# AIS-Bonn/stillleben

Hardware: AMD Instinct MI355X
Metric: scenes/sec (settle + 640x480 6-ch GT render), 20-obj YCB-like (higher is better)
Workload: dtype f32; 1 GPU; C2: 20 of 21 procedural YCB-like objects (8k verts/16k tris, 1024^2 texture each) per scene; per step and GPU 32768 scenes are staged (random stack), settled (100 frames x 4 substeps), framed (camera, light, shadow matrix) and rendered at 640x480 (rgb, coord+depth, class, instance, normals; shadows on, SSAO on) -- all four stages inside the timed region; render_chunk=512, objects=20, settle_streams=1, render_streams=2, pair_contact_budget=0, parallelism=1 GPU

## Files before the change

### include/slhip.h

```cpp
#ifndef SLHIP_H
#define SLHIP_H

#include <stdint.h>

#ifdef __cplusplus
extern "C" {
#endif

#define SLHIP_ABI_VERSION 5
#define SLHIP_NUM_LIGHTS 3


typedef struct {
    float* d_env;
    float* d_irradiance;
    float* d_prefilter;
    float* d_brdf_lut;
    uint32_t env_size, env_levels;
    uint32_t irr_size;
    uint32_t pre_size, pre_levels;
    uint32_t lut_size;
} slhip_light_map;

typedef struct {
// ... 105 lines not shown
} slhip_render_out;

typedef struct {
    uint64_t* d_vis;
    float*    d_hdr;
    float*    d_ao;
    float*    d_shadow;
    uint32_t* d_queue;
    float*    d_lum;
    float*    d_clip;
    uint32_t* d_shadow_tiles;
    uint32_t  queue_capacity;
    uint32_t  shadow_res;
    uint32_t  n_clip_verts;
    uint32_t  shadow_lights;
    float*    d_vattr;
} slhip_render_scratch;

int slhip_render(const slhip_mesh_pool* pool,
                 const slhip_scene* d_scenes, const slhip_draw* d_draws,
                 const slhip_chunk* d_chunks, uint32_t n_scenes, uint32_t n_draws, uint32_t n_chunks,
                 uint32_t width, uint32_t height, uint32_t flags,
                 const float* d_depth_peel,
                 const slhip_render_out* out, const slhip_render_scratch* scratch,
                 void* stream);

int slhip_timing_enable(int on);
int slhip_render_timings(float* ms_out);
int slhip_render_ssao_skipped(const slhip_render_scratch* scratch, uint32_t n_scenes, uint32_t width, uint32_t height,
                              uint64_t counts[2], void* stream);
int slhip_render_ssao_level_tables(float rho[5], uint32_t counts[6], uint8_t taps[384]);
int slhip_render_ssao_levels(const slhip_render_scratch* scratch, uint32_t n_scenes, uint32_t width, uint32_t height,
                             uint64_t counts[8], void* stream);

int slhip_render_scratch_bytes(uint32_t n_scenes, uint32_t width, uint32_t height,
                               uint32_t shadow_res, uint32_t queue_capacity,
                               uint64_t bytes_out[7]);

typedef struct {
    uint32_t px_visib, px_all;
    int32_t  bbox_visib[4];
    int32_t  bbox_obj[4];
} slhip_object_stats;

#define SLHIP_OBJECT_STATS_CAPACITY 1

int slhip_render_object_stats_bytes(uint32_t n_scenes, uint32_t n_slots, uint32_t width, uint32_t height,
                                    uint64_t* worst_case_words);

int slhip_render_object_stats(const slhip_mesh_pool* pool,
                              const slhip_scene* d_scenes, const slhip_draw* d_draws,
                              const slhip_chunk* d_chunks, uint32_t n_scenes, uint32_t n_draws, uint32_t n_chunks,
                              uint32_t width, uint32_t height, const slhip_render_scratch* scratch,
                              uint32_t n_slots, uint64_t* d_words, uint64_t capacity_words,
                              slhip_object_stats* d_out, uint64_t* words_needed, void* stream);

typedef struct {
    int32_t  tile_box[4];
    uint64_t word_offset[2];
    uint64_t rle_offset[2];
    uint32_t rle_count[2];
} slhip_object_mask;

#define SLHIP_OBJECT_MASKS_CAPACITY 2

int slhip_render_object_masks_bytes(uint32_t n_scenes, uint32_t n_slots, uint32_t width, uint32_t height,
// ... 675 lines not shown
```

### stillleben_amd/_abi.py

```python
import ctypes as C
import os

import numpy as np

NUM_LIGHTS = 3
CHUNK_TRIS = 256

DRAW_HAS_BASE_TEX = 1
DRAW_VERTEX_COLORS = 2
DRAW_CASTS_SHADOW = 4
DRAW_ALPHA_TEST = 8
DRAW_NO_VERTEX_ID = 16
DRAW_HAS_NORMAL_TEX = 32
DRAW_HAS_MR_TEX = 64
DRAW_HAS_OCCLUSION_TEX = 128
DRAW_HAS_EMISSIVE_TEX = 256
DRAW_HAS_STICKER = 512
SAMPLER_DEFAULT = 0x10 | 0x20 | (2 << 6)

OUT_RGB = 0x01
OUT_COORD = 0x02
OUT_CLASS = 0x04
OUT_INSTANCE = 0x08
OUT_NORMALS = 0x10
# ... 407 lines not shown
    L.slhip_render_timings.argtypes = [C.POINTER(C.c_float * 8)]
    L.slhip_diff_sobel_valid.argtypes = [C.c_void_p, C.c_void_p, C.c_int, C.c_int, C.c_int, C.c_void_p, C.c_void_p]
    L.slhip_diff_dilate.argtypes = [C.c_void_p, C.c_void_p, C.c_void_p, C.c_int, C.c_int, C.c_int, C.c_void_p, C.c_void_p, C.c_void_p]
    L.slhip_diff_image_gradients.argtypes = [C.c_void_p, C.c_void_p, C.c_int, C.c_int, C.c_void_p, C.c_void_p, C.c_void_p]
    L.slhip_diff_pose_backward.argtypes = [C.c_void_p] * 7 + [C.c_int, C.c_int, C.c_int] + [C.c_void_p] * 4
    L.slhip_diff_pose_backward_batch.argtypes = [C.c_void_p] * 4 + [C.c_uint64] + [C.c_void_p] * 3 + [C.c_int] * 4 + [C.c_void_p] * 4
    L.slhip_diff_vertex_backward.argtypes = [C.c_void_p] * 8 + [C.c_int, C.c_int, C.c_int] + [C.c_void_p] * 4
    L.slhip_settle.argtypes = [C.c_void_p, C.c_uint32, C.c_void_p, C.c_void_p, C.c_void_p, C.c_void_p,
                               C.c_void_p, C.c_uint64, C.c_void_p]
    L.slhip_settle_status.argtypes = [C.c_void_p, C.c_uint32, C.c_void_p, C.POINTER(C.c_uint32), C.c_void_p]
    L.slhip_host_shadow_matrices.argtypes = [C.c_void_p, C.c_void_p, C.c_void_p]
    L.slhip_host_normal_matrix.argtypes = [C.c_void_p, C.c_void_p]
    L.slhip_host_convex_hull.argtypes = [C.c_void_p, C.c_uint32, C.c_void_p, C.c_uint32, C.POINTER(C.c_uint32)]
    L.slhip_host_fill_holes.argtypes = [C.c_void_p, C.c_uint32, C.c_uint32, C.c_uint32]
    L.slhip_records_count.argtypes = [C.c_void_p, C.c_uint32, C.c_void_p, C.c_void_p, C.POINTER(C.c_uint32), C.POINTER(C.c_uint32)]
    L.slhip_records_build_render.argtypes = [C.c_void_p, C.c_uint32, C.c_void_p, C.c_void_p, C.c_uint32, C.c_void_p, C.c_void_p,
                                             C.c_uint32, C.c_void_p, C.c_uint32]
    L.slhip_render_object_stats.argtypes = [
        C.POINTER(MeshPool), C.c_void_p, C.c_void_p, C.c_void_p, C.c_uint32, C.c_uint32, C.c_uint32, C.c_uint32, C.c_uint32,
        C.POINTER(RenderScratch), C.c_uint32, C.c_void_p, C.c_uint64, C.c_void_p, C.POINTER(C.c_uint64), C.c_void_p,
    ]
    L.slhip_render_object_stats_bytes.argtypes = [C.c_uint32, C.c_uint32, C.c_uint32, C.c_uint32, C.POINTER(C.c_uint64)]
    L.slhip_render_object_masks.argtypes = [
        C.POINTER(MeshPool), C.c_void_p, C.c_void_p, C.c_void_p, C.c_uint32, C.c_uint32, C.c_uint32, C.c_uint32, C.c_uint32,
        C.POINTER(RenderScratch), C.c_uint32, C.c_void_p, C.c_uint64, C.c_void_p, C.POINTER(C.c_uint64),
        C.c_void_p, C.c_void_p, C.c_uint64, C.POINTER(C.c_uint64), C.c_void_p,
    ]
    L.slhip_render_object_masks_bytes.argtypes = [C.c_uint32, C.c_uint32, C.c_uint32, C.c_uint32, C.POINTER(C.c_uint64),
                                                  C.POINTER(C.c_uint64)]
    L.slhip_object_masks_expand.argtypes = [C.c_void_p, C.c_void_p, C.c_uint32, C.c_uint32, C.c_uint32, C.c_uint32, C.c_uint32,
                                            C.c_void_p, C.c_uint64, C.c_void_p, C.c_void_p]
    L.slhip_render_ssao_skipped.argtypes = [C.c_void_p, C.c_uint32, C.c_uint32, C.c_uint32, C.POINTER(C.c_uint64 * 2), C.c_void_p]
    L.slhip_render_ssao_levels.argtypes = [C.c_void_p, C.c_uint32, C.c_uint32, C.c_uint32, C.POINTER(C.c_uint64 * 8), C.c_void_p]
    L.slhip_render_ssao_level_tables.argtypes = [C.POINTER(C.c_float * 5), C.POINTER(C.c_uint32 * 6), C.POINTER(C.c_uint8 * 384)]
    L.slhip_settle_caps.argtypes = [C.c_void_p, C.c_uint32, C.c_void_p, C.POINTER(C.c_uint64 * 10), C.c_void_p]
    L.slhip_settle_timing_enable.argtypes = [C.c_int]
    L.slhip_settle_timings.argtypes = [C.POINTER(C.c_float * 5), C.POINTER(C.c_uint32 * 5)]
    if hasattr(L, "slhip_settle_timing_every"):
        L.slhip_settle_timing_every.argtypes = [C.c_uint32]
        L.slhip_settle_timings_by_step.argtypes = [C.c_void_p, C.c_void_p, C.c_uint32, C.POINTER(C.c_uint32)]
    L.slhip_settle_scratch_bytes.argtypes = [C.c_uint32, C.c_void_p, C.POINTER(C.c_uint64)]
    L.slhip_overlap_any.argtypes = [C.c_void_p, C.c_uint32, C.c_void_p, C.c_void_p, C.c_void_p, C.c_void_p, C.c_void_p]
    L.slhip_light_map_floats.argtypes = [C.c_uint32] * 6 + [C.POINTER(C.c_uint64 * 4)]
    L.slhip_light_map_build.argtypes = [C.c_void_p, C.c_int, C.c_int, C.c_void_p, C.c_void_p]
    L.slhip_camera_model.argtypes = [C.c_void_p, C.c_void_p, C.c_void_p, C.c_uint32, C.c_int, C.c_int, C.c_void_p, C.c_void_p]
    if hasattr(L, "slhip_depth_sensor"):
        L.slhip_depth_sensor_check_params.argtypes = [C.c_void_p, C.c_uint32, C.c_int]
        L.slhip_depth_sensor_timing_enable.argtypes = [C.c_int]
        L.slhip_depth_sensor_timings.argtypes = [C.POINTER(C.c_float * 2)]
        L.slhip_depth_sensor_scratch_bytes.argtypes = [C.c_uint32, C.c_int, C.c_int, C.POINTER(C.c_uint64)]
        L.slhip_depth_sensor.argtypes = [C.c_void_p, C.c_uint32, C.c_void_p, C.c_uint32, C.c_uint32, C.c_int, C.c_int, C.c_void_p,
                                         C.c_void_p, C.c_void_p, C.c_void_p, C.c_void_p, C.c_void_p]
    if hasattr(L, "slhip_object_crops_select"):
        L.slhip_object_crops_check_params.argtypes = [C.c_void_p, C.c_int, C.c_int]
        L.slhip_object_crops_scratch_bytes.argtypes = [C.c_uint32, C.POINTER(C.c_uint64)]
        L.slhip_object_crops_select.argtypes = [C.c_void_p, C.c_void_p, C.c_uint32, C.c_uint32, C.c_int, C.c_int, C.c_void_p,
                                                C.c_uint64, C.c_void_p, C.POINTER(C.c_uint64), C.c_void_p]
        L.slhip_object_crops_gather.argtypes = [C.c_void_p, C.c_void_p, C.c_uint64, C.POINTER(RenderOut), C.c_uint32, C.c_int,
                                                C.c_int, C.c_void_p, C.c_void_p, C.c_uint32, C.POINTER(ObjectCropsOut), C.c_void_p]
        L.slhip_object_crops_timing_enable.argtypes = [C.c_int]
        L.slhip_object_crops_timings.argtypes = [C.POINTER(C.c_float * 2)]
    if hasattr(L, "slhip_object_points_select"):
        L.slhip_object_points_check_params.argtypes = [C.c_void_p, C.c_int, C.c_int]
        L.slhip_object_points_scratch_bytes.argtypes = [C.c_uint32, C.POINTER(C.c_uint64)]
        L.slhip_object_points_select.argtypes = [C.c_void_p, C.c_void_p, C.c_void_p, C.c_uint32, C.c_uint32, C.c_void_p,
                                                 C.c_uint64, C.c_void_p, C.POINTER(C.c_uint64), C.c_void_p]
# ... 90 lines not shown
```

### stillleben_amd/_engine.py

```python
import ctypes as C

import numpy as np
import torch

from . import _abi
from ._batch import HostPool, build_batch

SHADOW_RES = 2048
QUEUE_ITEMS_PER_SCENE = int(__import__('os').environ.get('SLHIP_QUEUE_ITEMS', 1 << 14))


def _ptr(t):
    return C.c_void_p(t.data_ptr()) if t is not None else C.c_void_p(0)


class RenderBuffers:

    def __init__(self, device, B, H, W, mask):
        self.B, self.H, self.W, self.mask = B, H, W, mask

        def mk(bit, shape, dtype):
            return torch.empty(shape, dtype=dtype, device=device) if mask & bit else None

        self.rgb = mk(_abi.OUT_RGB, (B, H, W, 4), torch.uint8)
# ... 80 lines not shown
                "shadow_ready": False,
            }
            if len(self._scratch) > 6:
                self._scratch.clear()
            self._scratch[key] = s
        a = _abi.RenderScratch()
        a.d_vis, a.d_hdr, a.d_ao, a.d_shadow, a.d_queue, a.d_lum = (
            _ptr(s["vis"]), _ptr(s["hdr"]), _ptr(s["ao"]), _ptr(s["shadow"]), _ptr(s["queue"]), _ptr(s["lum"]))
        a.d_shadow_tiles = _ptr(s["tiles"])
        a.queue_capacity = s["qcap"]
        a.shadow_res = SHADOW_RES
        a.shadow_lights = shadow_lights
        return a, s

    def ssao_skipped(self, buffers, W, H):
        keep = buffers._keepalive[0]
        a = _abi.RenderScratch()
        a.d_ao = _ptr(keep["ao"])
        out = (C.c_uint64 * 2)()
        stream = torch.cuda.current_stream(self.device).cuda_stream
        with torch.cuda.device(self.device):
            _abi.check(self.L.slhip_render_ssao_skipped(C.byref(a), buffers.B, W, H, C.byref(out), C.c_void_p(stream)), "slhip_render_ssao_skipped")
        return int(out[0]), int(out[1])

    def ssao_levels(self, buffers, W, H):
        keep = buffers._keepalive[0]
        a = _abi.RenderScratch()
        a.d_ao = _ptr(keep["ao"])
        out = (C.c_uint64 * 8)()
        stream = torch.cuda.current_stream(self.device).cuda_stream
        with torch.cuda.device(self.device):
            _abi.check(self.L.slhip_render_ssao_levels(C.byref(a), buffers.B, W, H, C.byref(out), C.c_void_p(stream)), "slhip_render_ssao_levels")
        return [int(v) for v in out[:6]], int(out[6]), int(out[7])

    def upload_records(self, arr):
        raw = np.frombuffer(arr.tobytes(), dtype=np.uint8) if arr.size else np.zeros(16, np.uint8)
        return torch.from_numpy(raw.copy()).to(self.device)

    def render(self, scenes, mask=_abi.OUT_ALL, ssao=True, shadows=True, depth_peel=None, predicate=None,
               buffers=None, keep_hdr=False, object_stats=False, object_masks=False):
        W, H = scenes[0]._viewport
        for s in scenes:
            if s._viewport != (W, H):
                raise ValueError("all scenes of a batch must share one viewport")
        if (object_stats or object_masks) and depth_peel is not None:
            raise ValueError("object_stats / object_masks cannot be combined with depth_peel: a peeled layer has no single whole silhouette")
        n_slots = None
        if object_stats or object_masks:
            n_slots = 1 + max((int(o.instance_index) for s in scenes for o in s._objects), default=0)
        want_rgb = bool(mask & _abi.OUT_RGB)
        srec, drec, crec = build_batch(scenes, self.pool, predicate, with_shadows=shadows and want_rgb)
        return self.render_records(srec, drec, crec, W, H, mask, ssao, shadows, depth_peel, buffers, keep_hdr,
                                   object_stats=object_stats, n_slots=n_slots, object_masks=object_masks)

    def render_records(self, srec, drec, crec, W, H, mask=_abi.OUT_ALL, ssao=True, shadows=True, depth_peel=None,
                       buffers=None, keep_hdr=False, object_stats=False, n_slots=None, stats_capacity=None,
                       object_masks=False, masks_capacity=None):
        if (object_stats or object_masks) and n_slots is None:
            n_slots = 1 + (int((drec["instance_index"] & 0xFFFF).max()) if len(drec) else 0)
        d_s, d_d, d_c = self.upload_records(srec), self.upload_records(drec), self.upload_records(crec)
        n_clip = int(drec["n_verts"].sum()) if len(drec) else 0
        on = (np.abs(srec["light_color"][:, :, :3]).sum(axis=2) > 0) & (np.abs(srec["light_dir"][:, :, :3]).sum(axis=2) > 0)
        lights = max(1, int(np.max(np.nonzero(on.any(axis=0))[0]) + 1)) if on.any() else 1
        buffers = self.render_device(d_s, d_d, d_c, len(srec), len(drec), len(crec), n_clip, W, H, mask, ssao, shadows,
                                     depth_peel, buffers, keep_hdr, shadow_lights=lights, object_stats=object_stats,
                                     n_slots=n_slots, stats_capacity=stats_capacity, object_masks=object_masks,
# ... 116 lines not shown
```

### stillleben_amd/csrc/slhip_render.hip

```cpp
#include <algorithm>
#include <cmath>
#include <cstring>
#include <vector>
#include <type_traits>
#include "slhip_common.h"
#include "slhip_cubemap.h"
#include "slhip_raster_walk.h"
#include "slhip_tile_queue.h"

#ifndef SLHIP_RENDER_WAVES
#define SLHIP_RENDER_WAVES 0
#endif
#ifndef SLHIP_SHADE_WAVES
#define SLHIP_SHADE_WAVES 0
#endif
#ifndef SLHIP_SSAO_WAVES
#define SLHIP_SSAO_WAVES 0
#endif
#if SLHIP_RENDER_WAVES > 0
#define SLHIP_LIGHT_KERNEL __attribute__((amdgpu_waves_per_eu(1, SLHIP_RENDER_WAVES)))
#else
#define SLHIP_LIGHT_KERNEL
#endif
#if SLHIP_RENDER_WAVES > 0
#define SLHIP_SHADOW_RASTER_KERNEL SLHIP_LIGHT_KERNEL
#else
#define SLHIP_SHADOW_RASTER_KERNEL __attribute__((amdgpu_waves_per_eu(6)))
#endif
#if SLHIP_SSAO_WAVES > 0
#define SLHIP_SSAO_KERNEL __attribute__((amdgpu_waves_per_eu(1, SLHIP_SSAO_WAVES)))
#else
#define SLHIP_SSAO_KERNEL
#endif
#if SLHIP_SHADE_WAVES > 0
#define SLHIP_SHADE_KERNEL __attribute__((amdgpu_waves_per_eu(1, SLHIP_SHADE_WAVES)))
#else
#define SLHIP_SHADE_KERNEL
#endif
namespace {

// ... 1980 lines not shown
        for (; k < n_taps; ++k) tap(k);
    }
    };
    if (w_is_z) taps(std::true_type{});
    else taps(std::false_type{});
    return 1.0f - occlusion / 64.0f;
}

__global__ __launch_bounds__(256) SLHIP_SSAO_KERNEL void k_ssao(const slhip_scene* __restrict__ scenes, unsigned n_scenes, int W, int H,
                                              const float* __restrict__ cam, const float* __restrict__ nrm,
                                              const float* __restrict__ zplane, float* __restrict__ ao,
                                              const float* __restrict__ kern)
{
    const size_t P = (size_t)W * H;
    const unsigned blocks_per_scene = (unsigned)((P + 255) / 256);
    unsigned scene, blk;
    if (!scene_block(blocks_per_scene, n_scenes, scene, blk)) return;
    const unsigned pix = blk * 256 + (threadIdx.x >> 6) + 4u * (threadIdx.x & 63u);
    if (pix >= P) return;
    const float* proj = scenes[scene].proj;
    const float* camS = zplane + (size_t)scene * ((size_t)(W + 2) * (H + 2));
    const size_t gp = (size_t)scene * P + pix;
    const int i = (int)(pix % (unsigned)W), j = (int)(pix / (unsigned)W);
    const float4 n4 = reinterpret_cast<const float4*>(nrm)[gp];
    if (n4.x == 0.0f && n4.y == 0.0f && n4.z == 0.0f) { ao[gp] = 1.0f; return; }
    ao[gp] = ssao_pixel<true>(proj, camS, W, H, i, j, n4, reinterpret_cast<const float4*>(cam)[gp], kern);
}

constexpr int kSsaoTile = 8;
constexpr int kSsaoLevels = 6;
constexpr float kSsaoRho[kSsaoLevels - 1] = {0.81f, 0.6f, 0.45f, 0.3f, 0.2f};
__constant__ float c_ssao_level_kernel[kSsaoLevels * 192];
struct SsaoLevelCounts { int n[kSsaoLevels]; };

__global__ __launch_bounds__(256) void k_ssao_mask(const slhip_scene* __restrict__ scenes, int W, int H,
                                                  const float2* __restrict__ tiles, unsigned char* __restrict__ skip, int dbg,
                                                  unsigned* __restrict__ drain_stats)
{
    extern __shared__ int s_sat[];
    const int TW = W / kSsaoTile, TH = H / kSsaoTile, SW = TW + 1;
    const unsigned scene = blockIdx.x;
    const float2* T = tiles + (size_t)scene * (TW * TH);
    unsigned char* S = skip + (size_t)scene * (TW * TH);
    const float* proj = scenes[scene].proj;
    if (scene == 0 && threadIdx.x < 2) drain_stats[threadIdx.x] = 0u;
    const bool persp = proj[1] == 0.0f && proj[3] == 0.0f && proj[4] == 0.0f && proj[7] == 0.0f &&
                       proj[12] == 0.0f && proj[13] == 0.0f && proj[14] == 1.0f && proj[15] == 0.0f && proj[0] > 0.0f && proj[5] > 0.0f;
    for (int k = threadIdx.x; k < (TH + 1) * SW; k += 256) {
        const int r = k / SW, c = k % SW;
        s_sat[k] = (r > 0 && c > 0) ? (int)(__float_as_uint(T[(r - 1) * TW + (c - 1)].y) & 1u) : 0;
    }
    __syncthreads();
    for (int r = threadIdx.x + 1; r <= TH; r += 256) { int acc = 0; for (int c = 1; c <= TW; ++c) { acc += s_sat[r * SW + c]; s_sat[r * SW + c] = acc; } }
    __syncthreads();
    for (int c = threadIdx.x + 1; c <= TW; c += 256) { int acc = 0; for (int r = 1; r <= TH; ++r) { acc += s_sat[r * SW + c]; s_sat[r * SW + c] = acc; } }
    __syncthreads();
    const float fx = proj[0] * 0.5f * (float)W, fy = proj[5] * 0.5f * (float)H;
    const float tx = (1.0f + fabsf(proj[2])) / proj[0], ty = (1.0f + fabsf(proj[6])) / proj[5];
    const float tmax = fmaxf(tx, ty);
    const float reach = fmaxf(fx, fy) * 0.1f * sqrtf(1.0f + tmax * tmax) * 1.001f;
    for (int k = threadIdx.x; k < TW * TH; k += 256) {
        const float2 t = T[k];
        const unsigned fl = __float_as_uint(t.y);
        int lvl = kSsaoLevels - 1, pass = 0;
        if (!(fl & 2u)) { lvl = 0; pass = 1; }
        else if (persp && !(fl & 1u) && t.x > 0.2f) {
            for (int j = kSsaoLevels - 2; j >= -1; --j) {
                const int R = (int)ceilf((j >= 0 ? kSsaoRho[j] : 1.0f) * reach / (t.x - 0.1f)) + 2;
                const int x0 = (k % TW) * kSsaoTile - R, x1 = (k % TW) * kSsaoTile + kSsaoTile - 1 + R;
                const int y0 = (k / TW) * kSsaoTile - R, y1 = (k / TW) * kSsaoTile + kSsaoTile - 1 + R;
                if (!(x0 >= 0 && y0 >= 0 && x1 < W && y1 < H)) break;
                const int ca = x0 / kSsaoTile, cb = x1 / kSsaoTile + 1, ra = y0 / kSsaoTile, rb = y1 / kSsaoTile + 1;
                const int others = s_sat[rb * SW + cb] - s_sat[ra * SW + cb] - s_sat[rb * SW + ca] + s_sat[ra * SW + ca];
                if (others != 0) break;
                if (j >= 0) lvl = j;
                else pass = 1;
            }
        }
        if (dbg == 1) { lvl = 0; pass = 1; }
        if (dbg == 2) lvl = kSsaoLevels - 1;
        S[k] = (unsigned char)(lvl << 1 | pass);
    }
}

__global__ __launch_bounds__(256) SLHIP_SSAO_KERNEL void k_ssao_tiled(const slhip_scene* __restrict__ scenes, unsigned n_scenes, int W, int H,
                                                    const float* __restrict__ cam, const float* __restrict__ nrm,
                                                    const float* __restrict__ zplane, float* __restrict__ ao,
                                                    const float* __restrict__ level_kern, SsaoLevelCounts level_n,
                                                    const unsigned char* __restrict__ skip, unsigned band_rows,
                                                    unsigned* __restrict__ drain_stats)
{
    __shared__ unsigned s_q[4][kSsaoLevels - 1][128];
    const unsigned bands = ((unsigned)H + band_rows - 1u) / band_rows;
    unsigned scene, rest;
    if (!scene_block(bands * 4u, n_scenes, scene, rest)) return;
    const unsigned band = rest >> 2, yc = rest & 3u, xc = threadIdx.x >> 6, lane = threadIdx.x & 63u;
    const size_t P = (size_t)W * H;
    const float* proj = scenes[scene].proj;
    const float* camS = zplane + (size_t)scene * ((size_t)(W + 2) * (H + 2));
    const int TW = W / kSsaoTile;
    const unsigned char* S = skip + (size_t)scene * ((size_t)TW * (H / kSsaoTile));
    const float4* N4 = reinterpret_cast<const float4*>(nrm) + (size_t)scene * P;
    const float4* C4 = reinterpret_cast<const float4*>(cam) + (size_t)scene * P;
    float* A = ao + (size_t)scene * P;
    unsigned* q = &s_q[xc][0][0];
    const unsigned y_first = band * band_rows, rows = min(band_rows, (unsigned)H - y_first);
    const unsigned per_row = (unsigned)W >> 2, total = (rows >> 2) * per_row;
    unsigned cnt[kSsaoLevels] = {};
    auto pixel_of = [&](unsigned ci) -> unsigned { return (y_first + yc + 4u * (ci / per_row)) * (unsigned)W + xc + 4u * (ci % per_row); };
    auto fetch = [&](unsigned ci, unsigned& pix, unsigned& lvl, float4& n4) {
        pix = 0; lvl = 0; n4 = make_float4(0.0f, 0.0f, 0.0f, 0.0f);
        if (ci < total) {
            pix = pixel_of(ci);
            const unsigned y = pix / (unsigned)W, x = pix % (unsigned)W;
            const unsigned b = S[(y >> 3) * (unsigned)TW + (x >> 3)];
            lvl = min(b >> 1, (unsigned)(kSsaoLevels - 1));
            if (lvl) n4 = N4[pix];
        }
    };
    unsigned pix_n, lvl_n; float4 n4_n;
    fetch(lane, pix_n, lvl_n, n4_n);
    unsigned c0 = 0;
    for (;;) {
        unsigned pix = 0, list = 0;
        bool valid = false;
#pragma unroll
        for (int l = 1; l < kSsaoLevels; ++l)
            if (cnt[l] >= 64u) list = (unsigned)l;
        if (list) {
#pragma unroll
            for (int l = 1; l < kSsaoLevels; ++l)
                if (list == (unsigned)l) { cnt[l] -= 64u; pix = q[(l - 1) * 128 + cnt[l] + lane]; }
            valid = true;
        } else if (c0 < total) {
            const unsigned px = pix_n, lvl = lvl_n;
            const float4 n4 = n4_n;
            const bool in = c0 + lane < total;
            c0 += 64u;
            fetch(c0 + lane, pix_n, lvl_n, n4_n);
            const bool need = in && lvl != 0u && !(n4.x == 0.0f && n4.y == 0.0f && n4.z == 0.0f);
            if (in && !need) A[px] = 1.0f;
#pragma unroll
            for (int l = 1; l < kSsaoLevels; ++l) {
                const bool mine = need && lvl == (unsigned)l;
                const unsigned long long m = __ballot(mine);
                if (mine) q[(l - 1) * 128 + cnt[l] + (unsigned)__popcll(m & ((1ull << lane) - 1ull))] = px;
                cnt[l] += (unsigned)__popcll(m);
            }
            __builtin_amdgcn_wave_barrier();
            continue;
        } else {
            unsigned room = 64u, p = lane, lowest = 0;
#pragma unroll
            for (int l = kSsaoLevels - 1; l >= 1; --l) {
                const unsigned take = min(cnt[l], room);
                if (take) {
                    if (!list) list = (unsigned)l;
                    lowest = (unsigned)l;
                    cnt[l] -= take;
                    room -= take;
                    if (!valid) {
                        if (p < take) { pix = q[(l - 1) * 128 + cnt[l] + p]; valid = true; }
                        else p -= take;
                    }
                }
            }
            if (!list) break;
            if (drain_stats && lane == 0u) {
                atomicAdd(&drain_stats[0], 1u);
                if (lowest != list) atomicAdd(&drain_stats[1], 1u);
            }
        }
        __builtin_amdgcn_wave_barrier();
        int n_taps = 0;
#pragma unroll
        for (int l = 1; l < kSsaoLevels; ++l)
            if (list == (unsigned)l) n_taps = level_n.n[l];
        if (valid) {
            const int i = (int)(pix % (unsigned)W), j = (int)(pix / (unsigned)W);
            A[pix] = ssao_pixel(proj, camS, W, H, i, j, N4[pix], C4[pix], level_kern + 192u * list, n_taps);
        }
        __builtin_amdgcn_wave_barrier();
    }
}

__global__ __launch_bounds__(256) SLHIP_LIGHT_KERNEL void k_ssao_apply(const slhip_scene* __restrict__ scenes, unsigned n_scenes, int W, int H,
                                                    const float* __restrict__ hdr_in, const float* __restrict__ ao,
                                                    const float* __restrict__ zplane, float* __restrict__ hdr_out,
                                                    const float* __restrict__ lum_scene, uint8_t* __restrict__ rgb,
                                                    const unsigned char* __restrict__ skip)
{
    const size_t P = (size_t)W * H;
    const unsigned blocks_per_scene = (unsigned)((P + 255) / 256);
    unsigned scene, blk;
    if (!scene_block(blocks_per_scene, n_scenes, scene, blk)) return;
    const unsigned pix = blk * 256 + threadIdx.x;
    if (pix >= P) return;
    const float* camS = zplane + (size_t)scene * ((size_t)(W + 2) * (H + 2));
    const float* aoS = ao + (size_t)scene * P;
    const size_t gp = (size_t)scene * P + pix;
    const int i = (int)(pix % (unsigned)W), j = (int)(pix / (unsigned)W);
    if (skip) {
        const int TW = W / kSsaoTile;
        const unsigned char* S = skip + (size_t)scene * ((size_t)TW * (H / kSsaoTile));
        const int xa = max(i - 2, 0) >> 3, xb = min(i + 1, W - 1) >> 3, ya = max(j - 2, 0) >> 3, yb = min(j + 1, H - 1) >> 3;
        const bool ones = (S[ya * TW + xa] & S[ya * TW + xb] & S[yb * TW + xa] & S[yb * TW + xb] & 1) != 0;
        if (__all(ones)) {
            const float4 h = reinterpret_cast<const float4*>(hdr_in)[gp];
            const float c4[4] = {h.x, h.y, h.z, h.w};
            if (hdr_out) reinterpret_cast<float4*>(hdr_out)[gp] = h;
            if (rgb) {
                const float manual = scenes[scene].manual_exposure;
                const float lum = (manual >= 0.0f) ? 0.0f : lum_scene[(size_t)scene * blocks_per_scene * 4];
                reinterpret_cast<uchar4*>(rgb)[gp] = tone_map_px(c4, manual, lum);
            }
// ... 176 lines not shown
                if (j < kSsaoLevels - 1 && !(1.001 * std::sqrt(x * x + y * y + z * z) > (double)kSsaoRho[j])) continue;
                for (int c = 0; c < 3; ++c) t.kern[j * 192 + 3 * n + c] = k_ssao_kernel_host[3 * k + c];
                t.taps[j * 64 + n] = (uint8_t)k;
                ++n;
            }
            t.count.n[j] = n;
        }
        return t;
    }();
    return tables;
}
}

extern "C" int slhip_render_ssao_level_tables(float rho[5], uint32_t counts[6], uint8_t taps[384])
{
    if (!rho || !counts || !taps) {
        slhip::set_error("slhip_render_ssao_level_tables: null argument");
        return -1;
    }
    const SsaoLevelTables& t = ssao_level_tables();
    for (int j = 0; j < kSsaoLevels - 1; ++j) rho[j] = kSsaoRho[j];
    for (int j = 0; j < kSsaoLevels; ++j) counts[j] = (uint32_t)t.count.n[j];
    memcpy(taps, t.taps, sizeof(t.taps));
    return 0;
}

static inline uint64_t ssao_tiles_per_scene(uint32_t w, uint32_t h) { return (uint64_t)((w + 7) / 8) * ((h + 7) / 8); }
static inline uint64_t ssao_tiles_offset(uint64_t B, uint32_t w, uint32_t h)
{
    const uint64_t b = B * (uint64_t)w * h * 4 + B * (uint64_t)(w + 2) * (h + 2) * 4;
    return (b + 7u) & ~(uint64_t)7u;
}

constexpr uint64_t kSsaoScratchSpare = 16;
static_assert(7 + 2 * sizeof(unsigned) <= kSsaoScratchSpare, "the two counters of k_ssao_tiled, 8-byte aligned, live in the spare bytes");
static inline uint64_t ssao_stats_offset(uint64_t B, uint32_t w, uint32_t h)
{
    return (ssao_tiles_offset(B, w, h) + B * ssao_tiles_per_scene(w, h) * 9 + 7u) & ~(uint64_t)7u;
}

extern "C" int slhip_render_scratch_bytes(uint32_t n_scenes, uint32_t width, uint32_t height,
                                          uint32_t shadow_res, uint32_t queue_capacity, uint64_t bytes_out[7])
{
    const uint64_t P = (uint64_t)width * height, B = n_scenes;
    const uint64_t blocks = (P + 255) / 256;
    bytes_out[0] = B * P * 8;
    bytes_out[1] = 2 * B * P * 16;
    bytes_out[2] = ssao_tiles_offset(B, width, height) + B * ssao_tiles_per_scene(width, height) * 9 + kSsaoScratchSpare;
    bytes_out[3] = B * SLHIP_NUM_LIGHTS * (uint64_t)shadow_res * shadow_res * 4;
    bytes_out[4] = 16 + (uint64_t)queue_capacity * 16;
    bytes_out[5] = B * blocks * 16;
    bytes_out[6] = B * SLHIP_NUM_LIGHTS * (uint64_t)shadow_tile_words((int)shadow_res) * 4;
    return 0;
}

extern "C" int slhip_render_ssao_skipped(const slhip_render_scratch* scratch, uint32_t n_scenes, uint32_t width, uint32_t height,
                                         uint64_t counts[2], void* stream_)
{
    hipStream_t stream = (hipStream_t)stream_;
    if (!scratch || !scratch->d_ao || !counts) {
        slhip::set_error("slhip_render_ssao_skipped: null argument");
        return -1;
    }
    counts[0] = counts[1] = 0;
    if (width % 32 != 0 || height % 16 != 0 || n_scenes == 0) return 0;
    const uint64_t nt = (uint64_t)n_scenes * ssao_tiles_per_scene(width, height);
    std::vector<unsigned char> h(nt);
    const char* base = reinterpret_cast<const char*>(scratch->d_ao) + ssao_tiles_offset(n_scenes, width, height) + nt * 8;
    SLHIP_CHECK(hipMemcpyAsync(h.data(), base, nt, hipMemcpyDeviceToHost, stream));
    SLHIP_CHECK(hipStreamSynchronize(stream));
    counts[0] = nt;
    for (unsigned char b : h) counts[1] += b & 1;
    return 0;
}

extern "C" int slhip_render_ssao_levels(const slhip_render_scratch* scratch, uint32_t n_scenes, uint32_t width, uint32_t height,
                                        uint64_t counts[8], void* stream_)
{
    hipStream_t stream = (hipStream_t)stream_;
    if (!scratch || !scratch->d_ao || !counts) {
        slhip::set_error("slhip_render_ssao_levels: null argument");
        return -1;
    }
    for (int i = 0; i < 8; ++i) counts[i] = 0;
    if (width % 32 != 0 || height % 16 != 0 || n_scenes == 0) return 0;
    const uint64_t nt = (uint64_t)n_scenes * ssao_tiles_per_scene(width, height);
    std::vector<unsigned char> h(nt);
    unsigned stats[2] = {0, 0};
    const char* ao = reinterpret_cast<const char*>(scratch->d_ao);
    SLHIP_CHECK(hipMemcpyAsync(h.data(), ao + ssao_tiles_offset(n_scenes, width, height) + nt * 8, nt, hipMemcpyDeviceToHost, stream));
    SLHIP_CHECK(hipMemcpyAsync(stats, ao + ssao_stats_offset(n_scenes, width, height), sizeof(stats), hipMemcpyDeviceToHost, stream));
    SLHIP_CHECK(hipStreamSynchronize(stream));
    for (unsigned char b : h) counts[std::min<int>(b >> 1, kSsaoLevels - 1)] += 1;
    counts[6] = stats[0];
    counts[7] = stats[1];
    return 0;
}

constexpr int kSsaoBandRows = 16;
static unsigned ssao_band_rows_knob()
{
    const char* e = getenv("SLHIP_SSAO_BAND_ROWS");
    const int v = e ? atoi(e) : kSsaoBandRows;
    return (unsigned)std::min(std::max(16, v / 16 * 16), 1 << 16);
}

extern "C" int slhip_render(const slhip_mesh_pool* pool, const slhip_scene* d_scenes, const slhip_draw* d_draws,
                            const slhip_chunk* d_chunks, uint32_t n_scenes, uint32_t n_draws, uint32_t n_chunks,
                            uint32_t width,
                            uint32_t height, uint32_t flags, const float* d_depth_peel,
                            const slhip_render_out* out, const slhip_render_scratch* scratch, void* stream_)
{
    hipStream_t stream = (hipStream_t)stream_;
    if (!pool || !d_scenes || !d_draws || !out || !scratch) {
        slhip::set_error("slhip_render: null argument");
        return -1;
    }
    if (n_scenes == 0 || width == 0 || height == 0) return 0;
    if (!scratch->d_vis || !scratch->d_queue) {
        slhip::set_error("slhip_render: d_vis and d_queue scratch are required");
        return -1;
    }
    const bool want_rgb = out->d_rgb != nullptr;
    const bool ssao = (flags & SLHIP_RENDER_SSAO) && want_rgb;
    const bool shadows = (flags & SLHIP_RENDER_SHADOWS) && want_rgb && scratch->d_shadow != nullptr;
    if (shadows && (!scratch->d_shadow_tiles || (scratch->shadow_res & 3u))) {
        slhip::set_error("slhip_render: shadows need the d_shadow_tiles scratch and a shadow_res that is a multiple of 4");
        return -1;
// ... 123 lines not shown
    float2* ssao_tiles = ssao_tiled ? reinterpret_cast<float2*>(reinterpret_cast<char*>(scratch->d_ao) + ssao_tiles_offset(n_scenes, W, H)) : nullptr;
    unsigned char* ssao_skip = ssao_tiled ? reinterpret_cast<unsigned char*>(ssao_tiles + (size_t)n_scenes * ssao_tiles_per_scene(W, H)) : nullptr;
    const int shade_reference = getenv("SLHIP_SHADE_REFERENCE") ? atoi(getenv("SLHIP_SHADE_REFERENCE")) : 0;
    auto launch_shade = [&](auto kernel) {
        kernel<<<pix_blocks, 256, 0, stream>>>(*pool, d_scenes, d_draws, prm,
                                               reinterpret_cast<const unsigned long long*>(scratch->d_vis), *out, hdr0,
                                               shadows ? scratch->d_shadow : nullptr, scratch->d_lum, clipbuf,
                                               ssao ? scratch->d_ao + (size_t)n_scenes * P : nullptr, vattr, ssao_tiles,
                                               shadows && !getenv("SLHIP_NO_PCF_TILES") ? scratch->d_shadow_tiles : nullptr);
    };
    if (shade_reference) launch_shade(k_shade<true>);
    else launch_shade(k_shade<false>);
    SLHIP_LAUNCH_CHECK();
    if (shadows && n_chunks > 0) {
        k_shadow_restore<<<n_tile_words, 256, 0, stream>>>(reinterpret_cast<unsigned*>(scratch->d_shadow), scratch->d_shadow_tiles,
                                                          S, n_tile_words, NL);
        SLHIP_LAUNCH_CHECK();
    }

    if (want_rgb) {
        k_lum_reduce<<<n_scenes, 256, 0, stream>>>(d_scenes, (unsigned)((P + 255) / 256), P, scratch->d_lum);
        if (ssao) {
            mark(5, stream);
            const float* zpl = scratch->d_ao + (size_t)n_scenes * P;
            const float* d_kernel_table = nullptr;
            SLHIP_CHECK(hipGetSymbolAddress((void**)&d_kernel_table, HIP_SYMBOL(c_ssao_kernel)));
            if (ssao_tiled) {
                const unsigned band_rows = ssao_band_rows_knob();
                const int ssao_dbg = getenv("SLHIP_SSAO_DEBUG") ? atoi(getenv("SLHIP_SSAO_DEBUG")) : 0;
                const unsigned bands = ((unsigned)H + band_rows - 1u) / band_rows;
                unsigned* drain_stats = reinterpret_cast<unsigned*>(reinterpret_cast<char*>(scratch->d_ao) + ssao_stats_offset(n_scenes, W, H));
                const float* d_level_table = nullptr;
                SLHIP_CHECK(hipGetSymbolAddress((void**)&d_level_table, HIP_SYMBOL(c_ssao_level_kernel)));
                k_ssao_mask<<<n_scenes, 256, (size_t)(W / 8 + 1) * (H / 8 + 1) * 4, stream>>>(d_scenes, W, H, ssao_tiles, ssao_skip, ssao_dbg, drain_stats);
                k_ssao_tiled<<<8u * ((n_scenes + 7u) / 8u) * bands * 4u, 256, 0, stream>>>(d_scenes, n_scenes, W, H, out->d_cam_coord, out->d_normals,
                                                                                   zpl, scratch->d_ao, d_level_table, ssao_level_tables().count, ssao_skip,
                                                                                   band_rows, ssao_dbg == 3 ? drain_stats : nullptr);
            } else
                k_ssao<<<pix_blocks, 256, 0, stream>>>(d_scenes, n_scenes, W, H, out->d_cam_coord, out->d_normals, zpl, scratch->d_ao,
                                                       d_kernel_table);
            mark(6, stream);
            k_ssao_apply<<<pix_blocks, 256, 0, stream>>>(d_scenes, n_scenes, W, H, hdr0, scratch->d_ao, zpl,
                                                         (flags & SLHIP_RENDER_KEEP_HDR) ? hdr1 : nullptr, scratch->d_lum, out->d_rgb, ssao_skip);
            mark(7, stream);
        } else {
            mark(7, stream);
            k_tonemap<<<pix_blocks, 256, 0, stream>>>(d_scenes, n_scenes, W, H, hdr0, scratch->d_lum, out->d_rgb);
        }
        SLHIP_LAUNCH_CHECK();
    }
    mark(kNumPhases, stream);
    return 0;
}

#include "slhip_render_stats.inc"
#include "slhip_render_masks.inc"
```

Before: 11110 scenes/s.

## Pool leftover SSAO queue tails across waves in a block before draining

In the tiled SSAO kernel, each wave no longer drains its own partial per-level pixel queues. Instead, all four waves publish their leftover counts to shared memory, synchronise, and then cooperatively process the pooled leftovers as full 64-lane batches ordered by level. This is meant to reduce partially filled wave iterations and mixed-level drains at the tail of each band, at the cost of a block-wide barrier and extra indexing work. The change also skips the enqueue ballots when no lane needs SSAO, and adds debug counters plus a host query for run-slot statistics.

```diff
diff --git a/include/slhip.h b/include/slhip.h
--- a/include/slhip.h
+++ b/include/slhip.h
@@ -161,6 +161,8 @@
 int slhip_render_ssao_level_tables(float rho[5], uint32_t counts[6], uint8_t taps[384]);
 int slhip_render_ssao_levels(const slhip_render_scratch* scratch, uint32_t n_scenes, uint32_t width, uint32_t height,
                              uint64_t counts[8], void* stream);
+int slhip_render_ssao_run_slots(const slhip_render_scratch* scratch, uint32_t n_scenes, uint32_t width, uint32_t height,
+                                uint64_t slots[4], void* stream);
 
 int slhip_render_scratch_bytes(uint32_t n_scenes, uint32_t width, uint32_t height,
                                uint32_t shadow_res, uint32_t queue_capacity,
diff --git a/stillleben_amd/_abi.py b/stillleben_amd/_abi.py
--- a/stillleben_amd/_abi.py
+++ b/stillleben_amd/_abi.py
@@ -463,6 +463,7 @@
                                             C.c_void_p, C.c_uint64, C.c_void_p, C.c_void_p]
     L.slhip_render_ssao_skipped.argtypes = [C.c_void_p, C.c_uint32, C.c_uint32, C.c_uint32, C.POINTER(C.c_uint64 * 2), C.c_void_p]
     L.slhip_render_ssao_levels.argtypes = [C.c_void_p, C.c_uint32, C.c_uint32, C.c_uint32, C.POINTER(C.c_uint64 * 8), C.c_void_p]
+    L.slhip_render_ssao_run_slots.argtypes = [C.c_void_p, C.c_uint32, C.c_uint32, C.c_uint32, C.POINTER(C.c_uint64 * 4), C.c_void_p]
     L.slhip_render_ssao_level_tables.argtypes = [C.POINTER(C.c_float * 5), C.POINTER(C.c_uint32 * 6), C.POINTER(C.c_uint8 * 384)]
     L.slhip_settle_caps.argtypes = [C.c_void_p, C.c_uint32, C.c_void_p, C.POINTER(C.c_uint64 * 10), C.c_void_p]
     L.slhip_settle_timing_enable.argtypes = [C.c_int]
diff --git a/stillleben_amd/_engine.py b/stillleben_amd/_engine.py
--- a/stillleben_amd/_engine.py
+++ b/stillleben_amd/_engine.py
@@ -136,6 +136,16 @@
         with torch.cuda.device(self.device):
             _abi.check(self.L.slhip_render_ssao_levels(C.byref(a), buffers.B, W, H, C.byref(out), C.c_void_p(stream)), "slhip_render_ssao_levels")
         return [int(v) for v in out[:6]], int(out[6]), int(out[7])
+
+    def ssao_run_slots(self, buffers, W, H):
+        keep = buffers._keepalive[0]
+        a = _abi.RenderScratch()
+        a.d_ao = _ptr(keep["ao"])
+        out = (C.c_uint64 * 4)()
+        stream = torch.cuda.current_stream(self.device).cuda_stream
+        with torch.cuda.device(self.device):
+            _abi.check(self.L.slhip_render_ssao_run_slots(C.byref(a), buffers.B, W, H, C.byref(out), C.c_void_p(stream)), "slhip_render_ssao_run_slots")
+        return tuple(int(v) for v in out)
 
     def upload_records(self, arr):
         raw = np.frombuffer(arr.tobytes(), dtype=np.uint8) if arr.size else np.zeros(16, np.uint8)
diff --git a/stillleben_amd/csrc/slhip_render.hip b/stillleben_amd/csrc/slhip_render.hip
--- a/stillleben_amd/csrc/slhip_render.hip
+++ b/stillleben_amd/csrc/slhip_render.hip
@@ -6,6 +6,7 @@
 #include "slhip_common.h"
 #include "slhip_cubemap.h"
 #include "slhip_raster_walk.h"
+#include "slhip_ssao_pool.h"
 #include "slhip_tile_queue.h"
 
 #ifndef SLHIP_RENDER_WAVES
@@ -2052,6 +2053,7 @@
 constexpr float kSsaoRho[kSsaoLevels - 1] = {0.81f, 0.6f, 0.45f, 0.3f, 0.2f};
 __constant__ float c_ssao_level_kernel[kSsaoLevels * 192];
 struct SsaoLevelCounts { int n[kSsaoLevels]; };
+constexpr unsigned kSsaoStatWords = 2 + 2 * 4;
 
 __global__ __launch_bounds__(256) void k_ssao_mask(const slhip_scene* __restrict__ scenes, int W, int H,
                                                   const float2* __restrict__ tiles, unsigned char* __restrict__ skip, int dbg,
@@ -2063,7 +2065,7 @@
     const float2* T = tiles + (size_t)scene * (TW * TH);
     unsigned char* S = skip + (size_t)scene * (TW * TH);
     const float* proj = scenes[scene].proj;
-    if (scene == 0 && threadIdx.x < 2) drain_stats[threadIdx.x] = 0u;
+    if (scene == 0 && threadIdx.x < kSsaoStatWords) drain_stats[threadIdx.x] = 0u;
     const bool persp = proj[1] == 0.0f && proj[3] == 0.0f && proj[4] == 0.0f && proj[7] == 0.0f &&
                        proj[12] == 0.0f && proj[13] == 0.0f && proj[14] == 1.0f && proj[15] == 0.0f && proj[0] > 0.0f && proj[5] > 0.0f;
     for (int k = threadIdx.x; k < (TH + 1) * SW; k += 256) {
@@ -2108,9 +2110,11 @@
                                                     const float* __restrict__ zplane, float* __restrict__ ao,
                                                     const float* __restrict__ level_kern, SsaoLevelCounts level_n,
                                                     const unsigned char* __restrict__ skip, unsigned band_rows,
-                                                    unsigned* __restrict__ drain_stats)
-{
+                                                    unsigned* __restrict__ drain_stats, int pool)
+{
+    static_assert(slhip_sp::kWaves == 4 && slhip_sp::kLevels == kSsaoLevels - 1 && slhip_sp::kQueueWords == 128, "slhip_ssao_pool.h describes s_q");
     __shared__ unsigned s_q[4][kSsaoLevels - 1][128];
+    __shared__ unsigned s_left[slhip_sp::kSegments];
     const unsigned bands = ((unsigned)H + band_rows - 1u) / band_rows;
     unsigned scene, rest;
     if (!scene_block(bands * 4u, n_scenes, scene, rest)) return;
@@ -2140,9 +2144,39 @@
     };
     unsigned pix_n, lvl_n; float4 n4_n;
     fetch(lane, pix_n, lvl_n, n4_n);
+    auto run_taps = [&](unsigned pix, bool valid, unsigned list) {
+        int n_taps = 0;
+#pragma unroll
+        for (int l = 1; l < kSsaoLevels; ++l)
+            if (list == (unsigned)l) n_taps = level_n.n[l];
+        if (valid) {
+            const int i = (int)(pix % (unsigned)W), j = (int)(pix / (unsigned)W);
+            A[pix] = ssao_pixel(proj, camS, W, H, i, j, N4[pix], C4[pix], level_kern + 192u * list, n_taps);
+        }
+    };
+    auto count_drain_run = [&](unsigned list, bool valid, unsigned own) {
+        unsigned lowest = list, needed = 0;
+#pragma unroll
+        for (int l = kSsaoLevels - 1; l >= 1; --l) {
+            const unsigned n = (unsigned)__popcll(__ballot(valid && own == (unsigned)l));
+            if (n) lowest = (unsigned)l;
+            needed += n * (unsigned)level_n.n[l];
+        }
+        if (lane == 0u) {
+            unsigned long long* wide = reinterpret_cast<unsigned long long*>(drain_stats + 2);
+            unsigned issued = 0;
+#pragma unroll
+            for (int l = 1; l < kSsaoLevels; ++l)
+                if (list == (unsigned)l) issued = 64u * (unsigned)level_n.n[l];
+            atomicAdd(&drain_stats[0], 1u);
+            if (lowest != list) atomicAdd(&drain_stats[1], 1u);
+            atomicAdd(&wide[2], (unsigned long long)issued);
+            atomicAdd(&wide[3], (unsigned long long)needed);
+        }
+    };
     unsigned c0 = 0;
     for (;;) {
-        unsigned pix = 0, list = 0;
+        unsigned pix = 0, list = 0, own = 0;
         bool valid = false;
 #pragma unroll
         for (int l = 1; l < kSsaoLevels; ++l)
@@ -2152,6 +2186,15 @@
             for (int l = 1; l < kSsaoLevels; ++l)
                 if (list == (unsigned)l) { cnt[l] -= 64u; pix = q[(l - 1) * 128 + cnt[l] + lane]; }
             valid = true;
+            if (drain_stats && lane == 0u) {
+                unsigned long long* wide = reinterpret_cast<unsigned long long*>(drain_stats + 2);
+                unsigned issued = 0;
+#pragma unroll
+                for (int l = 1; l < kSsaoLevels; ++l)
+                    if (list == (unsigned)l) issued = 64u * (unsigned)level_n.n[l];
+                atomicAdd(&wide[0], 1ull);
+                atomicAdd(&wide[1], (unsigned long long)issued);
+            }
         } else if (c0 < total) {
             const unsigned px = pix_n, lvl = lvl_n;
             const float4 n4 = n4_n;
@@ -2160,47 +2203,59 @@
             fetch(c0 + lane, pix_n, lvl_n, n4_n);
             const bool need = in && lvl != 0u && !(n4.x == 0.0f && n4.y == 0.0f && n4.z == 0.0f);
             if (in && !need) A[px] = 1.0f;
-#pragma unroll
-            for (int l = 1; l < kSsaoLevels; ++l) {
-                const bool mine = need && lvl == (unsigned)l;
-                const unsigned long long m = __ballot(mine);
-                if (mine) q[(l - 1) * 128 + cnt[l] + (unsigned)__popcll(m & ((1ull << lane) - 1ull))] = px;
-                cnt[l] += (unsigned)__popcll(m);
+            if (__ballot(need) != 0ull) {
+#pragma unroll
+                for (int l = 1; l < kSsaoLevels; ++l) {
+                    const bool mine = need && lvl == (unsigned)l;
+                    const unsigned long long m = __ballot(mine);
+                    if (mine) q[(l - 1) * 128 + cnt[l] + (unsigned)__popcll(m & ((1ull << lane) - 1ull))] = px;
+                    cnt[l] += (unsigned)__popcll(m);
+                }
             }
             __builtin_amdgcn_wave_barrier();
             continue;
+        } else if (pool) {
+            break;
         } else {
-            unsigned room = 64u, p = lane, lowest = 0;
+            unsigned room = 64u, p = lane;
 #pragma unroll
             for (int l = kSsaoLevels - 1; l >= 1; --l) {
                 const unsigned take = min(cnt[l], room);
                 if (take) {
                     if (!list) list = (unsigned)l;
-                    lowest = (unsigned)l;
                     cnt[l] -= take;
                     room -= take;
                     if (!valid) {
-                        if (p < take) { pix = q[(l - 1) * 128 + cnt[l] + p]; valid = true; }
+                        if (p < take) { pix = q[(l - 1) * 128 + cnt[l] + p]; valid = true; own = (unsigned)l; }
                         else p -= take;
                     }
                 }
             }
             if (!list) break;
-            if (drain_stats && lane == 0u) {
-                atomicAdd(&drain_stats[0], 1u);
-                if (lowest != list) atomicAdd(&drain_stats[1], 1u);
-            }
+            if (drain_stats) count_drain_run(list, valid, own);
         }
         __builtin_amdgcn_wave_barrier();
-        int n_taps = 0;
-#pragma unroll
-        for (int l = 1; l < kSsaoLevels; ++l)
-            if (list == (unsigned)l) n_taps = level_n.n[l];
-        if (valid) {
-            const int i = (int)(pix % (unsigned)W), j = (int)(pix / (unsigned)W);
-            A[pix] = ssao_pixel(proj, camS, W, H, i, j, N4[pix], C4[pix], level_kern + 192u * list, n_taps);
-        }
+        run_taps(pix, valid, list);
         __builtin_amdgcn_wave_barrier();
+    }
+    if (!pool) return;
+    if (lane == 0u) {
+#pragma unroll
+        for (int l = 1; l < kSsaoLevels; ++l) s_left[xc * slhip_sp::kLevels + (unsigned)(l - 1)] = cnt[l];
+    }
+    __syncthreads();
+    unsigned left[slhip_sp::kSegments];
+#pragma unroll
+    for (unsigned s = 0; s < slhip_sp::kSegments; ++s) left[s] = __builtin_amdgcn_readfirstlane(s_left[s]);
+    const unsigned pooled = slhip_sp::total(left);
+    const unsigned* q_all = &s_q[0][0][0];
+    for (unsigned first = 64u * (unsigned)__builtin_amdgcn_readfirstlane(xc); first < pooled; first += 64u * slhip_sp::kWaves) {
+        unsigned list, own, word, word0;
+        slhip_sp::locate(left, first, list, word0);
+        const bool valid = slhip_sp::locate(left, first + lane, own, word);
+        const unsigned pix = valid ? q_all[word] : 0u;
+        if (drain_stats) count_drain_run(list, valid, own);
+        run_taps(pix, valid, list);
     }
 }
 
@@ -2443,8 +2498,8 @@
     return (b + 7u) & ~(uint64_t)7u;
 }
 
-constexpr uint64_t kSsaoScratchSpare = 16;
-static_assert(7 + 2 * sizeof(unsigned) <= kSsaoScratchSpare, "the two counters of k_ssao_tiled, 8-byte aligned, live in the spare bytes");
+constexpr uint64_t kSsaoScratchSpare = 48;
+static_assert(7 + kSsaoStatWords * sizeof(unsigned) <= kSsaoScratchSpare, "the counters of k_ssao_tiled, 8-byte aligned, live in the spare bytes");
 static inline uint64_t ssao_stats_offset(uint64_t B, uint32_t w, uint32_t h)
 {
     return (ssao_tiles_offset(B, w, h) + B * ssao_tiles_per_scene(w, h) * 9 + 7u) & ~(uint64_t)7u;
@@ -2505,6 +2560,24 @@
     for (unsigned char b : h) counts[std::min<int>(b >> 1, kSsaoLevels - 1)] += 1;
     counts[6] = stats[0];
     counts[7] = stats[1];
+    return 0;
+}
+
+extern "C" int slhip_render_ssao_run_slots(const slhip_render_scratch* scratch, uint32_t n_scenes, uint32_t width, uint32_t height,
+                                           uint64_t slots[4], void* stream_)
+{
+    hipStream_t stream = (hipStream_t)stream_;
+    if (!scratch || !scratch->d_ao || !slots) {
+        slhip::set_error("slhip_render_ssao_run_slots: null argument");
+        return -1;
+    }
+    for (int i = 0; i < 4; ++i) slots[i] = 0;
+    if (width % 32 != 0 || height % 16 != 0 || n_scenes == 0) return 0;
+    unsigned long long wide[4] = {0, 0, 0, 0};
+    const char* ao = reinterpret_cast<const char*>(scratch->d_ao);
+    SLHIP_CHECK(hipMemcpyAsync(wide, ao + ssao_stats_offset(n_scenes, width, height) + 2 * sizeof(unsigned), sizeof(wide), hipMemcpyDeviceToHost, stream));
+    SLHIP_CHECK(hipStreamSynchronize(stream));
+    for (int i = 0; i < 4; ++i) slots[i] = wide[i];
     return 0;
 }
 
@@ -2694,10 +2767,11 @@
                 unsigned* drain_stats = reinterpret_cast<unsigned*>(reinterpret_cast<char*>(scratch->d_ao) + ssao_stats_offset(n_scenes, W, H));
                 const float* d_level_table = nullptr;
                 SLHIP_CHECK(hipGetSymbolAddress((void**)&d_level_table, HIP_SYMBOL(c_ssao_level_kernel)));
+                const int ssao_pool = getenv("SLHIP_SSAO_POOL") ? atoi(getenv("SLHIP_SSAO_POOL")) : 1;
                 k_ssao_mask<<<n_scenes, 256, (size_t)(W / 8 + 1) * (H / 8 + 1) * 4, stream>>>(d_scenes, W, H, ssao_tiles, ssao_skip, ssao_dbg, drain_stats);
                 k_ssao_tiled<<<8u * ((n_scenes + 7u) / 8u) * bands * 4u, 256, 0, stream>>>(d_scenes, n_scenes, W, H, out->d_cam_coord, out->d_normals,
                                                                                    zpl, scratch->d_ao, d_level_table, ssao_level_tables().count, ssao_skip,
-                                                                                   band_rows, ssao_dbg == 3 ? drain_stats : nullptr);
+                                                                                   band_rows, ssao_dbg == 3 ? drain_stats : nullptr, ssao_pool != 0);
             } else
                 k_ssao<<<pix_blocks, 256, 0, stream>>>(d_scenes, n_scenes, W, H, out->d_cam_coord, out->d_normals, zpl, scratch->d_ao,
                                                        d_kernel_table);
diff --git a/stillleben_amd/csrc/slhip_ssao_pool.h b/stillleben_amd/csrc/slhip_ssao_pool.h
--- /dev/null
+++ b/stillleben_amd/csrc/slhip_ssao_pool.h
@@ -0,0 +1,48 @@
+#pragma once
+
+#if defined(__HIPCC__)
+#define SLHIP_SP_HD __host__ __device__ __forceinline__
+#else
+#define SLHIP_SP_HD inline
+#endif
+
+namespace slhip_sp {
+
+constexpr unsigned kWaves = 4;
+constexpr unsigned kLevels = 5;
+constexpr unsigned kSegments = kWaves * kLevels;
+constexpr unsigned kQueueWords = 128;
+
+SLHIP_SP_HD unsigned segment_wave(unsigned s) { return s % kWaves; }
+SLHIP_SP_HD unsigned segment_level(unsigned s) { return kLevels - s / kWaves; }
+SLHIP_SP_HD unsigned segment_count_index(unsigned s) { return segment_wave(s) * kLevels + (segment_level(s) - 1u); }
+SLHIP_SP_HD unsigned segment_queue_offset(unsigned s) { return segment_count_index(s) * kQueueWords; }
+
+SLHIP_SP_HD unsigned total(const unsigned* counts)
+{
+    unsigned t = 0;
+    for (unsigned s = 0; s < kSegments; ++s) t += counts[s];
+    return t;
+}
+
+SLHIP_SP_HD bool locate(const unsigned* counts, unsigned pos, unsigned& level, unsigned& word)
+{
+    bool found = false;
+    level = 0;
+    word = 0;
+#if defined(__HIPCC__)
+#pragma unroll
+#endif
+    for (unsigned s = 0; s < kSegments; ++s) {
+        const unsigned len = counts[segment_count_index(s)];
+        if (!found && pos < len) {
+            found = true;
+            level = segment_level(s);
+            word = segment_queue_offset(s) + pos;
+        }
+        pos -= len;
+    }
+    return found;
+}
+
+}
```

Measured after the change: 11280 scenes/s, median of 6. 1.02x the previous value.
